# gargatik/Seamless-Through-Breaking-Rethinking-Image-Stitching-for-Optimal-Alignment

Hardware: AMD Instinct MI355X
Metric: stitched image-pairs/s at 512x512 (higher is better)
Workload: dtype f32 (decoder contractions, PatchEmbed's third conv and the C = 128 block tails: exact 3xbf16 split of both operands, 6 products on the bf16 matrix cores, fp32 accumulate -- error vs fp64 0.83x the fp32 MFMA chain's; everything else fp32); 1 GPU; UDIS-D-shaped 512x512 pairs, batch=1, FlowHomoAdpater.forward(type=test_eval); launch=hipGraph replay, pairs_in_flight=3

## Files before the change

include/stitch_gfx950.h:

```cpp
#ifndef STITCH_GFX950_H
#define STITCH_GFX950_H
#include <stdint.h>
#ifdef __cplusplus
extern "C" {
#endif

typedef struct st_gemm_desc {
    const float* a;
    const float* w;
    float* c;
    const float* bias;
    const float* aux0;
    const float* aux1;
    const float* aux2;
    const float* scale_ptr;
    int32_t M, N, K;
    int32_t H, W, Cin, ldx;
    int32_t kh, kw, sh, sw, ph, pw, Ho, Wo;
    int32_t ldw, ldc, ld_aux0, ld_aux1, ld_aux2;
    int32_t aux0_row_div, aux0_row_mod;
    int32_t act;
    int32_t epi;
    float alpha;
    int32_t batch;
// ... 130 lines not shown
int st_coords_grid_init(float* out, const float* init, int32_t B, int32_t H, int32_t W, void* stream);
int st_flow_forward_interpolate(const float* src, int32_t src_is_coords_rows, float* out, int32_t B, int32_t H, int32_t W,
                                void* stream);
int st_flow_from_coords(const float* coords1, float* flow4, int32_t ld4, float* dst2, int32_t ld2, int32_t B,
                        int32_t H, int32_t W, void* stream);
int st_flow_encode(const float* coords1, const float* w98, const float* bias, float* out, int32_t ldo, float* flow2,
                   int32_t ld2, int32_t B, int32_t H, int32_t W, int32_t Co, void* stream);
int st_flow_encode_split3(const float* coords1, const float* w98, const float* bias, float* out, int32_t ldo, float* flow2,
                          int32_t ld2, int32_t B, int32_t H, int32_t W, int32_t Co, void* out_planes, int64_t out_pstride,
                          int64_t out_prows, void* flow_planes, int64_t flow_pstride, int64_t flow_prows, int32_t flow_col,
                          void* stream);
int st_cost_lookup(const float* maps, const float* coords, float* out, int32_t ldo, int32_t Nq, int32_t H2,
                   int32_t W2, int32_t r, void* stream);
int st_decoder_token_chain(float* corr, int32_t ld_corr, const float* coords1, const float* kv,
                           const float* const* weights16, int32_t rows, int32_t ntok, void* stream);
int st_convex_upsample(const float* coords1, const float* mask, int32_t ldm, float* out, int32_t B, int32_t H,
                       int32_t W, void* stream);

int st_dlt4(const float* src4x2, const float* motion, float* H, int32_t B, float mscale_x, float mscale_y,
            float div, void* stream);
int st_mat3_sandwich(const float* L, const float* X, const float* R, float* out, int32_t B, int32_t invert,
                     void* stream);
int st_homo_warp(const float* U, const float* theta, float* out, int32_t* idx, int32_t B, int32_t C,
                 int32_t n_ones, int32_t H, int32_t W, int32_t oh, int32_t ow, void* stream);
int st_mesh_bounds(const float* H, float* out4, int32_t B, float width, float height, int32_t gw, int32_t gh,
                   void* stream);
int st_flow_warp(const float* x, const float* flow, const float* mul, float* out, int32_t B, int32_t C,
                 int32_t H, int32_t W, void* stream);
int st_homo_flow_warp(const float* image2, const float* H8, const float* flow, float* out6, float* overlap, float* Hi,
                      int32_t B, int32_t H, int32_t W, void* stream);
// ... 133 lines not shown
```

seamless-through-breaking-rethinking-image-stitching-for-optimal-alignment_amd/csrc/flowops.hip:

```cpp
#include "common.h"
#include <type_traits>
#include "../../include/stitch_gfx950.h"

__global__ void coords_grid_kernel(float* __restrict__ out, int B, int H, int W) {
    const size_t idx = (size_t)blockIdx.x * blockDim.x + threadIdx.x;
    if (idx >= (size_t)B * H * W) return;
    const int r = idx % ((size_t)H * W);
    out[idx * 2] = (float)(r % W);
    out[idx * 2 + 1] = (float)(r / W);
}

extern "C" int st_coords_grid(float* out, int32_t B, int32_t H, int32_t W, void* stream) {
    if (!out || B <= 0 || H <= 0 || W <= 0) return ST_EINVAL;
    const size_t total = (size_t)B * H * W;
    hipLaunchKernelGGL(coords_grid_kernel, dim3((total + 255) / 256), dim3(256), 0, (hipStream_t)stream, out, B, H, W);
    ST_CHECK_LAUNCH();
    return ST_OK;
}

__global__ void coords_grid_init_kernel(float* __restrict__ out, const float* __restrict__ init, int B, int H, int W) {
    const size_t idx = (size_t)blockIdx.x * blockDim.x + threadIdx.x;
    if (idx >= (size_t)B * H * W) return;
    const size_t N = (size_t)H * W, b = idx / N;
    const int r = idx % N;
// ... 21 lines not shown
        for (int c = 2; c < ld4; ++c) flow4[idx * ld4 + c] = 0.f;
    }
    if (dst2) { dst2[idx * ld2] = fx; dst2[idx * ld2 + 1] = fy; }
}

extern "C" int st_flow_from_coords(const float* coords1, float* flow4, int32_t ld4, float* dst2, int32_t ld2, int32_t B,
                                   int32_t H, int32_t W, void* stream) {
    if (!coords1 || B <= 0 || H <= 0 || W <= 0 || (flow4 && ld4 < 2) || (dst2 && ld2 < 2)) return ST_EINVAL;
    const size_t total = (size_t)B * H * W;
    hipLaunchKernelGGL(flow_from_coords_kernel, dim3((total + 255) / 256), dim3(256), 0, (hipStream_t)stream, coords1, flow4,
                       ld4, dst2, ld2, B, H, W);
    ST_CHECK_LAUNCH();
    return ST_OK;
}

__global__ __launch_bounds__(512) void flow_encode_kernel(const float* __restrict__ coords1, const float* __restrict__ w,
                                                          const float* __restrict__ bias, float* __restrict__ out, int ldo,
                                                          float* __restrict__ flow2, int ld2, int H, int W, int Co,
                                                          __bf16* __restrict__ out_planes, long long out_pstride, long long out_prows,
                                                          __bf16* __restrict__ flow_planes, long long flow_pstride, long long flow_prows, int flow_col) {
    __shared__ float2 patch[10 * 14];
    __shared__ __attribute__((aligned(16))) float wsm[98 * 128];
    const int tid = threadIdx.x, lane = tid & 63, wave = __builtin_amdgcn_readfirstlane(tid >> 6);
    const int tiles_x = (W + 7) >> 3;
    const int b = blockIdx.z, ty = (int)blockIdx.x / tiles_x, tx = (int)blockIdx.x - ty * tiles_x;
    const size_t img = (size_t)b * H * W;
    const int cbase = (int)blockIdx.y * 128;
    {
        float4 v[7];
#pragma unroll
        for (int u = 0; u < 7; ++u) {
            const int f = u * 512 + tid, t = f >> 5, c4 = (f & 31) * 4;
            v[u] = make_float4(0.f, 0.f, 0.f, 0.f);
            if (t < 98 && cbase + c4 < Co) v[u] = *reinterpret_cast<const float4*>(w + (size_t)t * Co + cbase + c4);
        }
#pragma unroll
        for (int u = 0; u < 7; ++u) {
            const int f = u * 512 + tid;
            if (f < 98 * 32) *reinterpret_cast<float4*>(wsm + f * 4) = v[u];
        }
    }
    if (tid < 140) {
        const int py = tid / 14, px = tid - py * 14;
        const int y = ty * 4 + py - 3, x = tx * 8 + px - 3;
        float2 f = make_float2(0.f, 0.f);
        if (y >= 0 && y < H && x >= 0 && x < W) {
            const float2 cc = *reinterpret_cast<const float2*>(coords1 + (img + (size_t)y * W + x) * 2);
            f = make_float2(cc.x - (float)x, cc.y - (float)y);
        }
        patch[tid] = f;
    }
    __syncthreads();
    const int row = wave >> 1;
    const int y = ty * 4 + row;
    if (y >= H) return;
    const int cl = (wave & 1) * 64 + lane, c = cbase + cl;
    const bool cok = c < Co;
    const float bv = cok ? bias[c] : 0.f;
    float acc[8];
#pragma unroll
    for (int p = 0; p < 8; ++p) acc[p] = bv;
#pragma unroll 1
    for (int ky = 0; ky < 7; ++ky) {
        float2 f[14];
        float wr[14];
#pragma unroll
        for (int i = 0; i < 14; ++i) {
            f[i] = patch[(row + ky) * 14 + i];
            wr[i] = wsm[(ky * 14 + i) * 128 + cl];
        }
#pragma unroll
        for (int kx = 0; kx < 7; ++kx)
#pragma unroll
            for (int p = 0; p < 8; ++p) {
                acc[p] = fmaf(f[p + kx].x, wr[kx * 2], acc[p]);
                acc[p] = fmaf(f[p + kx].y, wr[kx * 2 + 1], acc[p]);
            }
    }
#pragma unroll
    for (int p = 0; p < 8; ++p) {
        const int x = tx * 8 + p;
        if (x < W && cok) {
            const float o = fmaxf(acc[p], 0.f);
            out[(img + (size_t)y * W + x) * ldo + c] = o;
            if (out_planes) {
                __bf16 h, m, l;
                st_split3(o, h, m, l);
                const unsigned ph = st_bf16_bits(h), pm = st_bf16_bits(m), pl = st_bf16_bits(l);
                const unsigned nh = (unsigned)__builtin_amdgcn_update_dpp(0, (int)ph, 0xB1, 0xF, 0xF, false);
                const unsigned nm = (unsigned)__builtin_amdgcn_update_dpp(0, (int)pm, 0xB1, 0xF, 0xF, false);
                const unsigned nl = (unsigned)__builtin_amdgcn_update_dpp(0, (int)pl, 0xB1, 0xF, 0xF, false);
                if (!(c & 1)) {
                    unsigned* pp = reinterpret_cast<unsigned*>(out_planes + ((size_t)(c >> 5) * out_prows + img + (size_t)y * W + x) * 32 + (c & 31));
                    pp[0] = ph | (nh << 16); pp[out_pstride / 2] = pm | (nm << 16); pp[out_pstride] = pl | (nl << 16);
                }
            }
        }
    }
    if (flow2 && blockIdx.y == 0 && (wave & 1) == 0 && lane < 8 && tx * 8 + lane < W) {
        const float2 f = patch[(row + 3) * 14 + lane + 3];
        const size_t r = img + (size_t)y * W + tx * 8 + lane;
        flow2[r * ld2] = f.x; flow2[r * ld2 + 1] = f.y;
        if (flow_planes) {
            __bf16 hx, mx, lx, hy, my, ly;
            unsigned* pp = reinterpret_cast<unsigned*>(flow_planes + ((size_t)(flow_col >> 5) * flow_prows + r) * 32 + (flow_col & 31));
            st_split3(f.x, hx, mx, lx);
            st_split3(f.y, hy, my, ly);
            pp[0] = st_bf16_bits(hx) | ((unsigned)st_bf16_bits(hy) << 16);
            pp[flow_pstride / 2] = st_bf16_bits(mx) | ((unsigned)st_bf16_bits(my) << 16);
            pp[flow_pstride] = st_bf16_bits(lx) | ((unsigned)st_bf16_bits(ly) << 16);
        }
    }
}

extern "C" int st_flow_encode(const float* coords1, const float* w98, const float* bias, float* out, int32_t ldo, float* flow2,
                              int32_t ld2, int32_t B, int32_t H, int32_t W, int32_t Co, void* stream) {
    if (!coords1 || !w98 || !bias || !out || B <= 0 || H <= 0 || W <= 0 || Co <= 0 || (Co & 3) || ((uintptr_t)w98 & 15)) return ST_EINVAL;
    if (ldo < Co || (flow2 && ld2 < 2) || ((uintptr_t)coords1 & 7)) return ST_EINVAL;
    dim3 grid(((H + 3) / 4) * ((W + 7) / 8), (Co + 127) / 128, B);
    hipLaunchKernelGGL(flow_encode_kernel, grid, dim3(512), 0, (hipStream_t)stream, coords1, w98, bias, out, ldo, flow2, ld2, H, W, Co,
                       (__bf16*)nullptr, 0LL, 0LL, (__bf16*)nullptr, 0LL, 0LL, 0);
    ST_CHECK_LAUNCH();
    return ST_OK;
}

extern "C" int st_flow_encode_split3(const float* coords1, const float* w98, const float* bias, float* out, int32_t ldo, float* flow2,
                                     int32_t ld2, int32_t B, int32_t H, int32_t W, int32_t Co, void* out_planes, int64_t out_pstride,
                                     int64_t out_prows, void* flow_planes, int64_t flow_pstride, int64_t flow_prows, int32_t flow_col,
                                     void* stream) {
    if (!coords1 || !w98 || !bias || !out || B <= 0 || H <= 0 || W <= 0 || Co <= 0 || (Co & 31) || ((uintptr_t)w98 & 15)) return ST_EINVAL;
    if (ldo < Co || (flow2 && ld2 < 2) || ((uintptr_t)coords1 & 7)) return ST_EINVAL;
    if (!out_planes || out_pstride <= 0 || out_prows < (int64_t)B * H * W) return ST_EINVAL;
    if (flow_planes && (!flow2 || flow_pstride <= 0 || flow_prows < (int64_t)B * H * W || flow_col < 0 || (flow_col & 1))) return ST_EINVAL;
    dim3 grid(((H + 3) / 4) * ((W + 7) / 8), (Co + 127) / 128, B);
    hipLaunchKernelGGL(flow_encode_kernel, grid, dim3(512), 0, (hipStream_t)stream, coords1, w98, bias, out, ldo, flow2, ld2, H, W, Co,
                       (__bf16*)out_planes, (long long)out_pstride, (long long)out_prows, (__bf16*)flow_planes, (long long)flow_pstride,
                       (long long)flow_prows, (int)flow_col);
    ST_CHECK_LAUNCH();
    return ST_OK;
}

__global__ __launch_bounds__(256) void cost_lookup_kernel(const float* __restrict__ maps, const float* __restrict__ coords,
                                                          float* __restrict__ out, int ldo, int Nq, int H2, int W2, int r) {
#pragma clang fp contract(off)
    const int side = 2 * r + 1, nch = side * side;
    const size_t idx = (size_t)blockIdx.x * 256 + threadIdx.x;
    if (idx >= (size_t)Nq * nch) return;
    const int ch = idx % nch;
    const size_t n = idx / nch;
    const int i = ch / side, j = ch % side;
    const float x = coords[n * 2] + (float)(i - r);
    const float y = coords[n * 2 + 1] + (float)(j - r);
    const float gx = 2.0f * x / (float)(W2 - 1) - 1.0f, gy = 2.0f * y / (float)(H2 - 1) - 1.0f;
    const float ix = ((gx + 1.0f) / 2.0f) * (float)(W2 - 1), iy = ((gy + 1.0f) / 2.0f) * (float)(H2 - 1);
    const float x0f = floorf(ix), y0f = floorf(iy);
    const int x0 = (int)x0f, y0 = (int)y0f, x1 = x0 + 1, y1 = y0 + 1;
    const float x1f = x0f + 1.0f, y1f = y0f + 1.0f;
    const float nw = (x1f - ix) * (y1f - iy), ne = (ix - x0f) * (y1f - iy);
    const float sw = (x1f - ix) * (iy - y0f), se = (ix - x0f) * (iy - y0f);
    const float* m = maps + n * (size_t)(H2 * W2);
    const bool xin0 = x0 >= 0 && x0 < W2, xin1 = x1 >= 0 && x1 < W2;
    const bool yin0 = y0 >= 0 && y0 < H2, yin1 = y1 >= 0 && y1 < H2;
    float v = (xin0 && yin0 ? m[y0 * W2 + x0] : 0.f) * nw;
    v = __fmaf_rn(xin1 && yin0 ? m[y0 * W2 + x1] : 0.f, ne, v);
    v = __fmaf_rn(xin0 && yin1 ? m[y1 * W2 + x0] : 0.f, sw, v);
    v = __fmaf_rn(xin1 && yin1 ? m[y1 * W2 + x1] : 0.f, se, v);
    out[n * ldo + ch] = v;
}

extern "C" int st_cost_lookup(const float* maps, const float* coords, float* out, int32_t ldo, int32_t Nq, int32_t H2,
                              int32_t W2, int32_t r, void* stream) {
    if (!maps || !coords || !out || Nq <= 0 || r < 0 || r > 64 || ldo < (2 * r + 1) * (2 * r + 1)) return ST_EINVAL;
    if (H2 < 2 || W2 < 2 || (int64_t)H2 * W2 > 0x7fffffff) return ST_EINVAL;
    const size_t total = (size_t)Nq * (2 * r + 1) * (2 * r + 1);
    hipLaunchKernelGGL(cost_lookup_kernel, dim3((total + 255) / 256), dim3(256), 0, (hipStream_t)stream, maps, coords, out,
                       ldo, Nq, H2, W2, r);
    ST_CHECK_LAUNCH();
    return ST_OK;
}

__global__ __launch_bounds__(256) void convex_upsample_kernel(const float* __restrict__ coords1, const float* __restrict__ mask,
                                                              int ldm, float* __restrict__ out, int B, int H, int W) {
// ... 98 lines not shown
    for (int r = 0; r < 4; ++r) {
        const float mo = red_other[(4 * g + r) * 2], m2o = red_other[(4 * g + r) * 2 + 1];
        const float mean = 0.5f * (mh[r] + mo), d = mh[r] - mo;
        const float var = ((m2h[r] + m2o) + d * d * 16.0f) * (1.0f / 64.0f);
        const float rstd = 1.0f / sqrtf(var + 1e-5f);
#pragma unroll
        for (int t = 0; t < 2; ++t) v[t][r] = (v[t][r] - mean) * rstd * w[col0 + 16 * t + c] + b[col0 + 16 * t + c];
    }
}

template <int I, int N, class F>
__device__ __forceinline__ void tc_static_for(F&& f) {
    if constexpr (I < N) { f(std::integral_constant<int, I>{}); tc_static_for<I + 1, N>(f); }
}

template <int RG>
__global__ __launch_bounds__(128 * RG) void decoder_token_chain_kernel(float* __restrict__ corr, int ldc, const float* __restrict__ coords1,
                                                                       const float* __restrict__ kv, TokenChainArgs A, int rows, int ntok) {
    extern __shared__ __attribute__((aligned(16))) float sm[];
    float* W0 = sm;
    float* W2 = W0 + 64 * TC_LDW0;
    float* Wq = W2 + 64 * TC_LDW;
    float* Wp = Wq + 64 * TC_LDW;
    float* Wf0 = Wp + 64 * TC_LDW;
    float* Wf3 = Wf0 + 64 * TC_LDW;
    float* Vec = Wf3 + 64 * TC_LDW;
    float* Slab = Vec + 10 * 64;
    float* Red = Slab + RG * 16 * (TC_LDW0 + TC_LDW);
    const int tid = threadIdx.x, lane = tid & 63, wave = tid >> 6;
    constexpr int NT = 128 * RG;
    const int rg = wave >> 1, hf = wave & 1, col0 = 32 * hf;
    float* S0 = Slab + rg * 16 * (TC_LDW0 + TC_LDW);
    float* S1 = S0 + 16 * TC_LDW0;
    float* red_mine = Red + (rg * 2 + hf) * 32;
    const float* red_other = Red + (rg * 2 + (hf ^ 1)) * 32;
    const int row0 = (blockIdx.x * RG + rg) * 16;
    const int c = lane & 15, g = lane >> 4;
    const int jmax = ntok - 1;

    constexpr int P0 = 1536 / NT, P1 = 1024 / NT;
    float4 xv[3], w0v[P0];
    f32x4 wv[5 * P1], vecv;
    float cx[4], cy[4];
    {
        const int e = min(tid, 159), q = e >> 4;
        const float* vp = q == 0 ? A.b0 : q == 1 ? A.b2 : q == 2 ? A.n1w : q == 3 ? A.n1b : q == 4 ? A.bq : q == 5 ? A.bp : q == 6 ? A.n2w
                          : q == 7 ? A.n2b : q == 8 ? A.bf0 : A.bf3;
        vecv = *reinterpret_cast<const f32x4*>(vp + 4 * (e & 15));
    }
    tc_static_for<0, 3>([&](auto ic) {
        constexpr int i = decltype(ic)::value;
        const int e = (hf * 64 + lane) + 128 * i, r = e / 24, k4 = e % 24;
        xv[i] = *reinterpret_cast<const float4*>(corr + (size_t)min(row0 + r, rows - 1) * ldc + 4 * min(k4, 20));
    });
    tc_static_for<0, P0>([&](auto ic) {
        constexpr int i = decltype(ic)::value;
        const int e = tid + NT * i, n = e / 24, k4 = e % 24;
        w0v[i] = *reinterpret_cast<const float4*>(A.w0 + n * 84 + 4 * min(k4, 20));
    });
    tc_static_for<0, P1>([&](auto ic) {
        constexpr int i = decltype(ic)::value;
        const int off = 4 * (tid + NT * i);
        wv[5 * i + 0] = *reinterpret_cast<const f32x4*>(A.w2 + off);
        wv[5 * i + 1] = *reinterpret_cast<const f32x4*>(A.wq + off);
        wv[5 * i + 2] = *reinterpret_cast<const f32x4*>(A.wp + off);
        wv[5 * i + 3] = *reinterpret_cast<const f32x4*>(A.wf0 + off);
        wv[5 * i + 4] = *reinterpret_cast<const f32x4*>(A.wf3 + off);
    });
#pragma unroll
    for (int r = 0; r < 4; ++r) {
        const float2 p2 = *reinterpret_cast<const float2*>(coords1 + (size_t)min(row0 + 4 * g + r, rows - 1) * 2);
        cx[r] = p2.x; cy[r] = p2.y;
    }
    tc_static_for<0, 3>([&](auto ic) {
        constexpr int i = decltype(ic)::value;
        const int e = (hf * 64 + lane) + 128 * i, r = e / 24, k4 = e % 24;
        *reinterpret_cast<float4*>(S0 + r * TC_LDW0 + 4 * k4) = k4 < 21 ? xv[i] : make_float4(0.f, 0.f, 0.f, 0.f);
    });
    tc_static_for<0, P0>([&](auto ic) {
        constexpr int i = decltype(ic)::value;
        const int e = tid + NT * i, n = e / 24, k4 = e % 24;
        *reinterpret_cast<float4*>(W0 + n * TC_LDW0 + 4 * k4) = k4 < 21 ? w0v[i] : make_float4(0.f, 0.f, 0.f, 0.f);
    });
    tc_static_for<0, P1>([&](auto ic) {
        constexpr int i = decltype(ic)::value;
        const int e = tid + NT * i, n = e >> 4, k4 = e & 15, off = n * TC_LDW + 4 * k4;
        *reinterpret_cast<f32x4*>(W2 + off) = wv[5 * i + 0];
        *reinterpret_cast<f32x4*>(Wq + off) = wv[5 * i + 1];
        *reinterpret_cast<f32x4*>(Wp + off) = wv[5 * i + 2];
        *reinterpret_cast<f32x4*>(Wf0 + off) = wv[5 * i + 3];
        *reinterpret_cast<f32x4*>(Wf3 + off) = wv[5 * i + 4];
    });
    if (tid < 160) *reinterpret_cast<f32x4*>(Vec + 4 * tid) = vecv;
    asm volatile("" ::: "memory");
    const int head = 4 * hf + g;
    float4 kk[8][2], vv[8][2];
    {
        const float* kvr = kv + (size_t)min(row0 + c, rows - 1) * ntok * 128 + 8 * head;
#pragma unroll
        for (int j = 0; j < 8; ++j)
#pragma unroll
            for (int e = 0; e < 2; ++e) kk[j][e] = *reinterpret_cast<const float4*>(kvr + min(j, jmax) * 128 + 4 * e);
#pragma unroll
        for (int j = 0; j < 8; ++j)
#pragma unroll
            for (int e = 0; e < 2; ++e) vv[j][e] = *reinterpret_cast<const float4*>(kvr + min(j, jmax) * 128 + 64 + 4 * e);
    }
    asm volatile("" ::: "memory");
// ... 82 lines not shown
    for (int t = 0; t < 2; ++t)
#pragma unroll
        for (int r = 0; r < 4; ++r) acc[t][r] = st_act(acc[t][r] + bf0[col0 + 16 * t + c], ST_ACT_GELU);
    tc_store2(S1, acc, col0, lane);
    __syncthreads();
    tc_gemm2<64, TC_LDW, TC_LDW>(S1, Wf3 + col0 * TC_LDW, acc, lane);
#pragma unroll
    for (int t = 0; t < 2; ++t)
#pragma unroll
        for (int r = 0; r < 4; ++r) {
            const int row = row0 + 4 * g + r;
            if (row < rows) corr[(size_t)row * ldc + 84 + col0 + 16 * t + c] = x[t][r] + (acc[t][r] + bf3[col0 + 16 * t + c]);
        }
}

extern "C" int st_decoder_token_chain(float* corr, int32_t ld_corr, const float* coords1, const float* kv, const float* const* weights16,
                                      int32_t rows, int32_t ntok, void* stream) {
    if (!corr || !coords1 || !kv || !weights16 || rows <= 0 || ntok <= 0 || ntok > 8 || ld_corr < 148 || (ld_corr & 3)) return ST_EINVAL;
    TokenChainArgs A;
    const float** dst = reinterpret_cast<const float**>(&A);
    for (int i = 0; i < 16; ++i) { if (!weights16[i]) return ST_EINVAL; dst[i] = weights16[i]; }
    constexpr int RG = 4;
    const size_t lds = (size_t)(64 * TC_LDW0 + 5 * 64 * TC_LDW + 640 + RG * 16 * (TC_LDW0 + TC_LDW) + RG * 64) * sizeof(float);
    (void)hipFuncSetAttribute((const void*)decoder_token_chain_kernel<RG>, hipFuncAttributeMaxDynamicSharedMemorySize, (int)lds);
    hipLaunchKernelGGL(decoder_token_chain_kernel<RG>, dim3((rows + 16 * RG - 1) / (16 * RG)), dim3(128 * RG), lds, (hipStream_t)stream, corr, ld_corr,
                       coords1, kv, A, rows, ntok);
    ST_CHECK_LAUNCH();
    return ST_OK;
}
```

seamless-through-breaking-rethinking-image-stitching-for-optimal-alignment_amd/flowformer.py:

```python
from __future__ import annotations

import os

import torch
import torch.nn as nn

from . import ops
from .checkpoint import HP, ParamTree, flat_params, flow_spec
from .homography import pack_conv


SPLIT3 = os.environ.get("ST_SPLIT3", "1") != "0"


def _new(rows, cols, dev, zero=False):
    return (torch.zeros if zero else torch.empty)((rows, cols), device=dev, dtype=torch.float32)


def _planes_copy(p):
    return ops.Planes(p.rows, p.C, None, t=p.t.clone(), c0=p.c0, ncols=p.ncols)


def _keep(trace, **named):
    if trace is None:
# ... 451 lines not shown
        for sfx in ("1", "2"):
            tabs[sfx] = _new(inp.shape[0], 384, inp.device)
            ops.conv_gemm(inp, D["inp" + sfx][0], tabs[sfx], geom=gru_geom[sfx], bias=D["inp" + sfx][1])
        return tabs

    def _update_state(self, R, B, N, dev):
        S = dict(hxA=_new(R, 384, dev), hxB=_new(R, 384, dev), corr=_new(R, 160, dev, zero=True),
                 cor1=_new(R, 256, dev), corflo=_new(R, 256, dev), flo1=_new(R, 128, dev),
                 vT=torch.empty((B, 128, N), device=dev), zbuf=_new(R, 128, dev), fh=_new(R, 256, dev))
        S["s3"] = SPLIT3 and N % 32 == 0 and "s3" in self._pk["dec"]
        if S["s3"]:
            S.update(hxA_p=ops.Planes(R, 384, dev), hxB_p=ops.Planes(R, 384, dev), cor1_p=ops.Planes(R, 256, dev), flo1_p=ops.Planes(R, 128, dev),
                     corflo_p=ops.Planes(R, 256, dev))
        return S

    def _update_block(self, S, coords1, attn, gru_tab, B, H1, W1, trace=None):
        D = self._pk["dec"]
        N = H1 * W1
        s3 = S["s3"]
        hxA = S["hxA"]
        net, motion, flow, agg = hxA[:, :128], hxA[:, 128:254], hxA[:, 254:256], hxA[:, 256:]
        g3 = (B, H1, W1, 3, 3, 1, 1, 1, 1)
        _keep(trace, coords_in=coords1, net_in=net)
        ops.conv_gemm(S["corr"], D["convc1"][0], S["cor1"], bias=D["convc1"][1], act="relu", **_emit(S, "cor1", 0, 256))
        enc = (coords1, D["convf1"][0], D["convf1"][1], S["flo1"], flow, B, H1, W1)
        if s3:
            ops.flow_encode_split3(*enc, S["flo1_p"], (S["hxA_p"], 254))
        else:
            ops.flow_encode(*enc)
        ops.conv_gemm_pair((_act(S, "cor1", 0, 256), _wt(D, S, "convc2"), S["corflo"][:, :192],
                            dict(geom=g3, bias=D["convc2"][1], act="relu", **_emit(S, "corflo", 0, 192, no_f32=True))),
                           (_act(S, "flo1", 0, 128), _wt(D, S, "convf2"), S["corflo"][:, 192:],
                            dict(geom=g3, bias=D["convf2"][1], act="relu", **_emit(S, "corflo", 192, 256, no_f32=True))))
        corflo = _act(S, "corflo", 0, 256)
        _keep(trace, cor1=S["cor1"], flo1=S["flo1"], flow=flow, **{"corflo_p" if s3 else "corflo": corflo})
        ops.conv_gemm(corflo, _wt(D, S, "conv"), motion, geom=g3, bias=D["conv"][1], act="relu", **_emit(S, "hxA", 128, 256))
        _keep(trace, motion=motion)
        ops.gma_aggregate(attn, hxA[:, 128:256], D["to_v"], D["gamma"], S["vT"], agg, B, N, **_emit(S, "hxA", 256, 384))
        _keep(trace, aggregate=agg)
        gru = (S["zbuf"], gru_tab["1"], gru_tab["2"], *((D["s3"] if s3 else D)[k] for k in ("zr1", "q1", "zr2", "q2")), B, H1, W1)
        if s3:
            ops.sepconv_gru_split3(hxA, S["hxA_p"], S["hxB_p"], *gru)
        else:
            ops.sepconv_gru(hxA, S["hxB"], *gru)
# ... 33 lines not shown
    def _decoder(self, mem, ctx, cost_maps, B, H1, W1, iters, trace=None, flow_init=None):
        D = self._pk["dec"]
        dev = ctx.device
        N = H1 * W1
        R = B * N
        nl = self._pk["latents"].shape[0]
        pro = None if trace is None else trace[-1].setdefault("prologue", {})
        pre = self._decoder_prologue(ctx, B, H1, W1, trace=pro)
        S, gru_tab, attn = pre["S"], pre["gru_tab"], pre["attn"]
        kv = _new(R * nl, 128, dev)
        ops.conv_gemm(mem, D["ca"]["kv"][0], kv, bias=D["ca"]["kv"][1])
        _keep(pro, kv=kv)
        coords1 = _new(R, 2, dev)
        ops.coords_grid(coords1, B, H1, W1, init=flow_init)
        for it in range(iters):
            ops.cost_lookup9x9(cost_maps, coords1, S["corr"], R, H1, W1)
            ops.decoder_token_chain(S["corr"], coords1, kv, D["chain16"], R, nl)
            rec = _record(trace)
            self._update_block(S, coords1, attn, gru_tab, B, H1, W1, trace=rec)
            _keep(rec, coords1=coords1, net=S["hxA"][:, :128], corr=S["corr"])
        last = None if trace is None else trace[-1]
        mask = self._mask_head(S, B, H1, W1, trace=last)
        flow_up = torch.empty((B, 2, 8 * H1, 8 * W1), device=dev)
        ops.convex_upsample(coords1, mask, flow_up, B, H1, W1)
        _keep(last, mask=mask, flow_up=flow_up)
        return flow_up, coords1

    def _forward(self, image1, image2, iters, trace, flow_init, pair):
        if not image1.is_cuda:
            raise RuntimeError("FlowFormer runs on the MI355X HIP kernels only: move the module and inputs to cuda")
        pk = self._pk or self.pack()
        iters = HP["decoder_depth"] if iters is None else iters
        B, _, H, W = image1.shape
        if H % 32 or W % 32:
            raise RuntimeError(f"input size {H}x{W} must be a multiple of 32 (reference runs both nets at 512x512)")
# ... 44 lines not shown
```

seamless-through-breaking-rethinking-image-stitching-for-optimal-alignment_amd/ops.py:

```python
from __future__ import annotations

import ctypes as C

import torch

from ._lib import ChainDesc, GemmDesc, MlpDesc, check, lib
from ._lib import StitchError as StitchErrorBase

ACT = dict(none=0, relu=1, gelu=2, sigmoid=3, tanh=4, lrelu=5)
EPI = dict(store=0, add=1, mul=2, gru=3, axpy=4, zr=5)

assert lib.st_abi_gemm_desc_size() == C.sizeof(GemmDesc), "st_gemm_desc ABI mismatch between header and binding"
assert lib.st_abi_chain_desc_size() == C.sizeof(ChainDesc), "st_chain_desc ABI mismatch between header and binding"
assert lib.st_abi_mlp_desc_size() == C.sizeof(MlpDesc), "st_mlp_desc ABI mismatch between header and binding"


def _stream():
    return C.c_void_p(torch.cuda.current_stream().cuda_stream)


def _p(t):
    if t is None:
        return None
    assert t.is_cuda, "device tensor expected (no CPU fallback)"
# ... 404 lines not shown
                                    C.c_void_p(fp.t.data_ptr()), fp.pstride, fp.rows, int(fcol), _stream()), "st_flow_encode_split3")
    return out


def cost_lookup(maps, coords, out, Nq, H2, W2, r=4):
    check(lib.st_cost_lookup(_p(maps), _p(coords), _p(out), _ld(out), Nq, H2, W2, r, _stream()), "st_cost_lookup")
    return out


def decoder_token_chain(corr, coords1, kv, weights16, rows, ntok):
    arr = (C.c_void_p * 16)(*[w.data_ptr() for w in weights16])
    check(lib.st_decoder_token_chain(_p(corr), _ld(corr), _pc(coords1), _p(kv), arr, rows, ntok, _stream()), "st_decoder_token_chain")
    return corr


def _ws(dev):
    ws = _workspace(dev)
    return ws.data_ptr(), ws.numel()


def patch_conv12(maps, c0_w, c0_b, c2_w, c2_b, out, M, H=64, W=64):
    check(lib.st_patch_conv12(_pc(maps), _pc(c0_w), _pc(c0_b), _pc(c2_w), _pc(c2_b), _p(out), M, H, W, _stream()), "st_patch_conv12")
    return out


def cost_lookup9x9(maps, coords, out, Nq, H2, W2):
    check(lib.st_cost_lookup9x9(_p(maps), _pc(coords), _p(out), _ld(out), Nq, H2, W2, _stream()), "st_cost_lookup9x9")
    return out


# ... 625 lines not shown
```

Baseline: 93.94 pairs/s.

## Fuse cost lookup, token chain and flow encode into one decoder-front kernel

```diff
diff --git a/include/stitch_gfx950.h b/include/stitch_gfx950.h
--- a/include/stitch_gfx950.h
+++ b/include/stitch_gfx950.h
@@ -168,6 +168,10 @@
                    int32_t W2, int32_t r, void* stream);
 int st_decoder_token_chain(float* corr, int32_t ld_corr, const float* coords1, const float* kv,
                            const float* const* weights16, int32_t rows, int32_t ntok, void* stream);
+int st_decoder_front(const float* cost_maps, const float* coords1, float* corr, int32_t ld_corr, const float* kv,
+                     const float* const* weights16, int32_t ntok, const float* w98, const float* bias, float* flo1, int32_t ld_flo1,
+                     float* flow2, int32_t ld2, int32_t B, int32_t H, int32_t W, void* flo1_planes, int64_t flo1_pstride,
+                     int64_t flo1_prows, void* flow_planes, int64_t flow_pstride, int64_t flow_prows, int32_t flow_col, void* stream);
 int st_convex_upsample(const float* coords1, const float* mask, int32_t ldm, float* out, int32_t B, int32_t H,
                        int32_t W, void* stream);
 
diff --git a/seamless-through-breaking-rethinking-image-stitching-for-optimal-alignment_amd/csrc/flowops.hip b/seamless-through-breaking-rethinking-image-stitching-for-optimal-alignment_amd/csrc/flowops.hip
--- a/seamless-through-breaking-rethinking-image-stitching-for-optimal-alignment_amd/csrc/flowops.hip
+++ b/seamless-through-breaking-rethinking-image-stitching-for-optimal-alignment_amd/csrc/flowops.hip
@@ -59,33 +59,33 @@
     return ST_OK;
 }
 
-__global__ __launch_bounds__(512) void flow_encode_kernel(const float* __restrict__ coords1, const float* __restrict__ w,
-                                                          const float* __restrict__ bias, float* __restrict__ out, int ldo,
-                                                          float* __restrict__ flow2, int ld2, int H, int W, int Co,
-                                                          __bf16* __restrict__ out_planes, long long out_pstride, long long out_prows,
-                                                          __bf16* __restrict__ flow_planes, long long flow_pstride, long long flow_prows, int flow_col) {
-    __shared__ float2 patch[10 * 14];
-    __shared__ __attribute__((aligned(16))) float wsm[98 * 128];
-    const int tid = threadIdx.x, lane = tid & 63, wave = __builtin_amdgcn_readfirstlane(tid >> 6);
-    const int tiles_x = (W + 7) >> 3;
-    const int b = blockIdx.z, ty = (int)blockIdx.x / tiles_x, tx = (int)blockIdx.x - ty * tiles_x;
-    const size_t img = (size_t)b * H * W;
-    const int cbase = (int)blockIdx.y * 128;
-    {
-        float4 v[7];
-#pragma unroll
-        for (int u = 0; u < 7; ++u) {
-            const int f = u * 512 + tid, t = f >> 5, c4 = (f & 31) * 4;
-            v[u] = make_float4(0.f, 0.f, 0.f, 0.f);
-            if (t < 98 && cbase + c4 < Co) v[u] = *reinterpret_cast<const float4*>(w + (size_t)t * Co + cbase + c4);
-        }
-#pragma unroll
-        for (int u = 0; u < 7; ++u) {
-            const int f = u * 512 + tid;
-            if (f < 98 * 32) *reinterpret_cast<float4*>(wsm + f * 4) = v[u];
-        }
-    }
+struct FlowEncArgs {
+    const float *w, *bias;
+    float* out; int ldo;
+    float* flow2; int ld2;
+    int H, W, Co;
+    __bf16* out_planes; long long out_pstride, out_prows;
+    __bf16* flow_planes; long long flow_pstride, flow_prows; int flow_col;
+};
+
+__device__ __forceinline__ void fe_stage_weights(float* __restrict__ wsm, const float* __restrict__ w, int cbase, int Co, int tid) {
+    float4 v[7];
+#pragma unroll
+    for (int u = 0; u < 7; ++u) {
+        const int f = u * 512 + tid, t = f >> 5, c4 = (f & 31) * 4;
+        v[u] = make_float4(0.f, 0.f, 0.f, 0.f);
+        if (t < 98 && cbase + c4 < Co) v[u] = *reinterpret_cast<const float4*>(w + (size_t)t * Co + cbase + c4);
+    }
+#pragma unroll
+    for (int u = 0; u < 7; ++u) {
+        const int f = u * 512 + tid;
+        if (f < 98 * 32) *reinterpret_cast<float4*>(wsm + f * 4) = v[u];
+    }
+}
+
+__device__ __forceinline__ void fe_stage_patch(float2* __restrict__ patch, const float* __restrict__ coords1, int b, int ty, int tx, int H, int W, int tid) {
     if (tid < 140) {
+        const size_t img = (size_t)b * H * W;
         const int py = tid / 14, px = tid - py * 14;
         const int y = ty * 4 + py - 3, x = tx * 8 + px - 3;
         float2 f = make_float2(0.f, 0.f);
@@ -95,13 +95,19 @@
         }
         patch[tid] = f;
     }
-    __syncthreads();
+}
+
+__device__ __forceinline__ void fe_tile(const float2* __restrict__ patch, const float* __restrict__ wsm, const FlowEncArgs& F, int b, int ty, int tx,
+                                        int cbase, int tid) {
+    const int lane = tid & 63, wave = __builtin_amdgcn_readfirstlane(tid >> 6);
+    const int H = F.H, W = F.W, Co = F.Co, ldo = F.ldo;
+    const size_t img = (size_t)b * H * W;
     const int row = wave >> 1;
     const int y = ty * 4 + row;
     if (y >= H) return;
     const int cl = (wave & 1) * 64 + lane, c = cbase + cl;
     const bool cok = c < Co;
-    const float bv = cok ? bias[c] : 0.f;
+    const float bv = cok ? F.bias[c] : 0.f;
     float acc[8];
 #pragma unroll
     for (int p = 0; p < 8; ++p) acc[p] = bv;
@@ -127,8 +133,8 @@
         const int x = tx * 8 + p;
         if (x < W && cok) {
             const float o = fmaxf(acc[p], 0.f);
-            out[(img + (size_t)y * W + x) * ldo + c] = o;
-            if (out_planes) {
+            F.out[(img + (size_t)y * W + x) * ldo + c] = o;
+            if (F.out_planes) {
                 __bf16 h, m, l;
                 st_split3(o, h, m, l);
                 const unsigned ph = st_bf16_bits(h), pm = st_bf16_bits(m), pl = st_bf16_bits(l);
@@ -136,26 +142,39 @@
                 const unsigned nm = (unsigned)__builtin_amdgcn_update_dpp(0, (int)pm, 0xB1, 0xF, 0xF, false);
                 const unsigned nl = (unsigned)__builtin_amdgcn_update_dpp(0, (int)pl, 0xB1, 0xF, 0xF, false);
                 if (!(c & 1)) {
-                    unsigned* pp = reinterpret_cast<unsigned*>(out_planes + ((size_t)(c >> 5) * out_prows + img + (size_t)y * W + x) * 32 + (c & 31));
-                    pp[0] = ph | (nh << 16); pp[out_pstride / 2] = pm | (nm << 16); pp[out_pstride] = pl | (nl << 16);
+                    unsigned* pp = reinterpret_cast<unsigned*>(F.out_planes + ((size_t)(c >> 5) * F.out_prows + img + (size_t)y * W + x) * 32 + (c & 31));
+                    pp[0] = ph | (nh << 16); pp[F.out_pstride / 2] = pm | (nm << 16); pp[F.out_pstride] = pl | (nl << 16);
                 }
             }
         }
     }
-    if (flow2 && blockIdx.y == 0 && (wave & 1) == 0 && lane < 8 && tx * 8 + lane < W) {
+    if (F.flow2 && cbase == 0 && (wave & 1) == 0 && lane < 8 && tx * 8 + lane < W) {
         const float2 f = patch[(row + 3) * 14 + lane + 3];
         const size_t r = img + (size_t)y * W + tx * 8 + lane;
-        flow2[r * ld2] = f.x; flow2[r * ld2 + 1] = f.y;
-        if (flow_planes) {
+        F.flow2[r * F.ld2] = f.x; F.flow2[r * F.ld2 + 1] = f.y;
+        if (F.flow_planes) {
             __bf16 hx, mx, lx, hy, my, ly;
-            unsigned* pp = reinterpret_cast<unsigned*>(flow_planes + ((size_t)(flow_col >> 5) * flow_prows + r) * 32 + (flow_col & 31));
+            unsigned* pp = reinterpret_cast<unsigned*>(F.flow_planes + ((size_t)(F.flow_col >> 5) * F.flow_prows + r) * 32 + (F.flow_col & 31));
             st_split3(f.x, hx, mx, lx);
             st_split3(f.y, hy, my, ly);
             pp[0] = st_bf16_bits(hx) | ((unsigned)st_bf16_bits(hy) << 16);
-            pp[flow_pstride / 2] = st_bf16_bits(mx) | ((unsigned)st_bf16_bits(my) << 16);
-            pp[flow_pstride] = st_bf16_bits(lx) | ((unsigned)st_bf16_bits(ly) << 16);
-        }
-    }
+            pp[F.flow_pstride / 2] = st_bf16_bits(mx) | ((unsigned)st_bf16_bits(my) << 16);
+            pp[F.flow_pstride] = st_bf16_bits(lx) | ((unsigned)st_bf16_bits(ly) << 16);
+        }
+    }
+}
+
+__global__ __launch_bounds__(512) void flow_encode_kernel(const float* __restrict__ coords1, FlowEncArgs F) {
+    __shared__ float2 patch[10 * 14];
+    __shared__ __attribute__((aligned(16))) float wsm[98 * 128];
+    const int tid = threadIdx.x;
+    const int tiles_x = (F.W + 7) >> 3;
+    const int b = blockIdx.z, ty = (int)blockIdx.x / tiles_x, tx = (int)blockIdx.x - ty * tiles_x;
+    const int cbase = (int)blockIdx.y * 128;
+    fe_stage_weights(wsm, F.w, cbase, F.Co, tid);
+    fe_stage_patch(patch, coords1, b, ty, tx, F.H, F.W, tid);
+    __syncthreads();
+    fe_tile(patch, wsm, F, b, ty, tx, cbase, tid);
 }
 
 extern "C" int st_flow_encode(const float* coords1, const float* w98, const float* bias, float* out, int32_t ldo, float* flow2,
@@ -163,8 +182,8 @@
     if (!coords1 || !w98 || !bias || !out || B <= 0 || H <= 0 || W <= 0 || Co <= 0 || (Co & 3) || ((uintptr_t)w98 & 15)) return ST_EINVAL;
     if (ldo < Co || (flow2 && ld2 < 2) || ((uintptr_t)coords1 & 7)) return ST_EINVAL;
     dim3 grid(((H + 3) / 4) * ((W + 7) / 8), (Co + 127) / 128, B);
-    hipLaunchKernelGGL(flow_encode_kernel, grid, dim3(512), 0, (hipStream_t)stream, coords1, w98, bias, out, ldo, flow2, ld2, H, W, Co,
-                       (__bf16*)nullptr, 0LL, 0LL, (__bf16*)nullptr, 0LL, 0LL, 0);
+    const FlowEncArgs F{w98, bias, out, ldo, flow2, ld2, H, W, Co, nullptr, 0, 0, nullptr, 0, 0, 0};
+    hipLaunchKernelGGL(flow_encode_kernel, grid, dim3(512), 0, (hipStream_t)stream, coords1, F);
     ST_CHECK_LAUNCH();
     return ST_OK;
 }
@@ -178,39 +197,57 @@
     if (!out_planes || out_pstride <= 0 || out_prows < (int64_t)B * H * W) return ST_EINVAL;
     if (flow_planes && (!flow2 || flow_pstride <= 0 || flow_prows < (int64_t)B * H * W || flow_col < 0 || (flow_col & 1))) return ST_EINVAL;
     dim3 grid(((H + 3) / 4) * ((W + 7) / 8), (Co + 127) / 128, B);
-    hipLaunchKernelGGL(flow_encode_kernel, grid, dim3(512), 0, (hipStream_t)stream, coords1, w98, bias, out, ldo, flow2, ld2, H, W, Co,
-                       (__bf16*)out_planes, (long long)out_pstride, (long long)out_prows, (__bf16*)flow_planes, (long long)flow_pstride,
-                       (long long)flow_prows, (int)flow_col);
-    ST_CHECK_LAUNCH();
-    return ST_OK;
+    const FlowEncArgs F{w98, bias, out, ldo, flow2, ld2, H, W, Co, (__bf16*)out_planes, (long long)out_pstride, (long long)out_prows,
+                        (__bf16*)flow_planes, (long long)flow_pstride, (long long)flow_prows, (int)flow_col};
+    hipLaunchKernelGGL(flow_encode_kernel, grid, dim3(512), 0, (hipStream_t)stream, coords1, F);
+    ST_CHECK_LAUNCH();
+    return ST_OK;
+}
+
+struct LookupTaps {
+    int x0, y0;
+    float nw, ne, sw, se;
+};
+
+__device__ __forceinline__ LookupTaps lookup_taps(float cx, float cy, int di, int dj, int H2, int W2) {
+#pragma clang fp contract(off)
+    const float x = cx + (float)di;
+    const float y = cy + (float)dj;
+    const float gx = 2.0f * x / (float)(W2 - 1) - 1.0f, gy = 2.0f * y / (float)(H2 - 1) - 1.0f;
+    const float ix = ((gx + 1.0f) / 2.0f) * (float)(W2 - 1), iy = ((gy + 1.0f) / 2.0f) * (float)(H2 - 1);
+    const float x0f = floorf(ix), y0f = floorf(iy);
+    const float x1f = x0f + 1.0f, y1f = y0f + 1.0f;
+    LookupTaps t;
+    t.x0 = (int)x0f; t.y0 = (int)y0f;
+    t.nw = (x1f - ix) * (y1f - iy); t.ne = (ix - x0f) * (y1f - iy);
+    t.sw = (x1f - ix) * (iy - y0f); t.se = (ix - x0f) * (iy - y0f);
+    return t;
+}
+
+__device__ __forceinline__ float lookup_blend(float vnw, float vne, float vsw, float vse, const LookupTaps& t) {
+#pragma clang fp contract(off)
+    float v = vnw * t.nw;
+    v = __fmaf_rn(vne, t.ne, v);
+    v = __fmaf_rn(vsw, t.sw, v);
+    v = __fmaf_rn(vse, t.se, v);
+    return v;
 }
 
 __global__ __launch_bounds__(256) void cost_lookup_kernel(const float* __restrict__ maps, const float* __restrict__ coords,
                                                           float* __restrict__ out, int ldo, int Nq, int H2, int W2, int r) {
-#pragma clang fp contract(off)
     const int side = 2 * r + 1, nch = side * side;
     const size_t idx = (size_t)blockIdx.x * 256 + threadIdx.x;
     if (idx >= (size_t)Nq * nch) return;
     const int ch = idx % nch;
     const size_t n = idx / nch;
     const int i = ch / side, j = ch % side;
-    const float x = coords[n * 2] + (float)(i - r);
-    const float y = coords[n * 2 + 1] + (float)(j - r);
-    const float gx = 2.0f * x / (float)(W2 - 1) - 1.0f, gy = 2.0f * y / (float)(H2 - 1) - 1.0f;
-    const float ix = ((gx + 1.0f) / 2.0f) * (float)(W2 - 1), iy = ((gy + 1.0f) / 2.0f) * (float)(H2 - 1);
-    const float x0f = floorf(ix), y0f = floorf(iy);
-    const int x0 = (int)x0f, y0 = (int)y0f, x1 = x0 + 1, y1 = y0 + 1;
-    const float x1f = x0f + 1.0f, y1f = y0f + 1.0f;
-    const float nw = (x1f - ix) * (y1f - iy), ne = (ix - x0f) * (y1f - iy);
-    const float sw = (x1f - ix) * (iy - y0f), se = (ix - x0f) * (iy - y0f);
+    const LookupTaps t = lookup_taps(coords[n * 2], coords[n * 2 + 1], i - r, j - r, H2, W2);
+    const int x0 = t.x0, y0 = t.y0, x1 = x0 + 1, y1 = y0 + 1;
     const float* m = maps + n * (size_t)(H2 * W2);
     const bool xin0 = x0 >= 0 && x0 < W2, xin1 = x1 >= 0 && x1 < W2;
     const bool yin0 = y0 >= 0 && y0 < H2, yin1 = y1 >= 0 && y1 < H2;
-    float v = (xin0 && yin0 ? m[y0 * W2 + x0] : 0.f) * nw;
-    v = __fmaf_rn(xin1 && yin0 ? m[y0 * W2 + x1] : 0.f, ne, v);
-    v = __fmaf_rn(xin0 && yin1 ? m[y1 * W2 + x0] : 0.f, sw, v);
-    v = __fmaf_rn(xin1 && yin1 ? m[y1 * W2 + x1] : 0.f, se, v);
-    out[n * ldo + ch] = v;
+    out[n * ldo + ch] = lookup_blend(xin0 && yin0 ? m[y0 * W2 + x0] : 0.f, xin1 && yin0 ? m[y0 * W2 + x1] : 0.f,
+                                     xin0 && yin1 ? m[y1 * W2 + x0] : 0.f, xin1 && yin1 ? m[y1 * W2 + x1] : 0.f, t);
 }
 
 extern "C" int st_cost_lookup(const float* maps, const float* coords, float* out, int32_t ldo, int32_t Nq, int32_t H2,
@@ -339,10 +376,10 @@
     if constexpr (I < N) { f(std::integral_constant<int, I>{}); tc_static_for<I + 1, N>(f); }
 }
 
-template <int RG>
-__global__ __launch_bounds__(128 * RG) void decoder_token_chain_kernel(float* __restrict__ corr, int ldc, const float* __restrict__ coords1,
-                                                                       const float* __restrict__ kv, TokenChainArgs A, int rows, int ntok) {
-    extern __shared__ __attribute__((aligned(16))) float sm[];
+template <int RG, bool LOOKUP>
+__device__ __forceinline__ void tc_body(float* __restrict__ sm, int wg, float* __restrict__ corr, int ldc, const float* __restrict__ coords1,
+                                        const float* __restrict__ kv, const TokenChainArgs& A, int rows, int ntok, const float* __restrict__ maps,
+                                        int mapH, int mapW) {
     float* W0 = sm;
     float* W2 = W0 + 64 * TC_LDW0;
     float* Wq = W2 + 64 * TC_LDW;
@@ -359,7 +396,7 @@
     float* S1 = S0 + 16 * TC_LDW0;
     float* red_mine = Red + (rg * 2 + hf) * 32;
     const float* red_other = Red + (rg * 2 + (hf ^ 1)) * 32;
-    const int row0 = (blockIdx.x * RG + rg) * 16;
+    const int row0 = (wg * RG + rg) * 16;
     const int c = lane & 15, g = lane >> 4;
     const int jmax = ntok - 1;
 
@@ -367,13 +404,24 @@
     float4 xv[3], w0v[P0];
     f32x4 wv[5 * P1], vecv;
     float cx[4], cy[4];
+    constexpr int LK = 11;
+    static_assert(!LOOKUP || NT == 8 * 16 * RG, "the lookup gives 8 threads to each of the workgroup's rows");
+    const int lrow = tid >> 3, lc0 = tid & 7;
+    const int lgrow = min(wg * RG * 16 + lrow, rows - 1);
+    float2 lxy = make_float2(0.f, 0.f);
+    if constexpr (LOOKUP) lxy = *reinterpret_cast<const float2*>(coords1 + (size_t)lgrow * 2);
+#pragma unroll
+    for (int r = 0; r < 4; ++r) {
+        const float2 p2 = *reinterpret_cast<const float2*>(coords1 + (size_t)min(row0 + 4 * g + r, rows - 1) * 2);
+        cx[r] = p2.x; cy[r] = p2.y;
+    }
     {
         const int e = min(tid, 159), q = e >> 4;
         const float* vp = q == 0 ? A.b0 : q == 1 ? A.b2 : q == 2 ? A.n1w : q == 3 ? A.n1b : q == 4 ? A.bq : q == 5 ? A.bp : q == 6 ? A.n2w
                           : q == 7 ? A.n2b : q == 8 ? A.bf0 : A.bf3;
         vecv = *reinterpret_cast<const f32x4*>(vp + 4 * (e & 15));
     }
-    tc_static_for<0, 3>([&](auto ic) {
+    if constexpr (!LOOKUP) tc_static_for<0, 3>([&](auto ic) {
         constexpr int i = decltype(ic)::value;
         const int e = (hf * 64 + lane) + 128 * i, r = e / 24, k4 = e % 24;
         xv[i] = *reinterpret_cast<const float4*>(corr + (size_t)min(row0 + r, rows - 1) * ldc + 4 * min(k4, 20));
@@ -392,12 +440,20 @@
         wv[5 * i + 3] = *reinterpret_cast<const f32x4*>(A.wf0 + off);
         wv[5 * i + 4] = *reinterpret_cast<const f32x4*>(A.wf3 + off);
     });
-#pragma unroll
-    for (int r = 0; r < 4; ++r) {
-        const float2 p2 = *reinterpret_cast<const float2*>(coords1 + (size_t)min(row0 + 4 * g + r, rows - 1) * 2);
-        cx[r] = p2.x; cy[r] = p2.y;
-    }
-    tc_static_for<0, 3>([&](auto ic) {
+    float tap[LK][4];
+    if constexpr (LOOKUP) {
+        const float* m = maps + (size_t)lgrow * (size_t)(mapH * mapW);
+        tc_static_for<0, LK>([&](auto kc) {
+            constexpr int k = decltype(kc)::value;
+            const int ch = min(lc0 + 8 * k, 80);
+            const LookupTaps t = lookup_taps(lxy.x, lxy.y, ch / 9 - 4, ch % 9 - 4, mapH, mapW);
+            const int xa = min(max(t.x0, 0), mapW - 1), xb = min(max(t.x0, -1), mapW - 2) + 1;
+            const int ya = min(max(t.y0, 0), mapH - 1), yb = min(max(t.y0, -1), mapH - 2) + 1;
+            tap[k][0] = m[ya * mapW + xa]; tap[k][1] = m[ya * mapW + xb];
+            tap[k][2] = m[yb * mapW + xa]; tap[k][3] = m[yb * mapW + xb];
+        });
+    }
+    if constexpr (!LOOKUP) tc_static_for<0, 3>([&](auto ic) {
         constexpr int i = decltype(ic)::value;
         const int e = (hf * 64 + lane) + 128 * i, r = e / 24, k4 = e % 24;
         *reinterpret_cast<float4*>(S0 + r * TC_LDW0 + 4 * k4) = k4 < 21 ? xv[i] : make_float4(0.f, 0.f, 0.f, 0.f);
@@ -417,6 +473,23 @@
         *reinterpret_cast<f32x4*>(Wf3 + off) = wv[5 * i + 4];
     });
     if (tid < 160) *reinterpret_cast<f32x4*>(Vec + 4 * tid) = vecv;
+    if constexpr (LOOKUP) {
+        float* Srow = Slab + (lrow >> 4) * 16 * (TC_LDW0 + TC_LDW) + (lrow & 15) * TC_LDW0;
+        const bool live = wg * RG * 16 + lrow < rows;
+        tc_static_for<0, LK>([&](auto kc) {
+            constexpr int k = decltype(kc)::value;
+            const int chr = lc0 + 8 * k, ch = min(chr, 80);
+            const LookupTaps t = lookup_taps(lxy.x, lxy.y, ch / 9 - 4, ch % 9 - 4, mapH, mapW);
+            const int x0 = t.x0, y0 = t.y0, x1 = x0 + 1, y1 = y0 + 1;
+            const bool xin0 = x0 >= 0 && x0 < mapW, xin1 = x1 >= 0 && x1 < mapW;
+            const bool yin0 = y0 >= 0 && y0 < mapH, yin1 = y1 >= 0 && y1 < mapH;
+            const float v = lookup_blend(xin0 && yin0 ? tap[k][0] : 0.f, xin1 && yin0 ? tap[k][1] : 0.f, xin0 && yin1 ? tap[k][2] : 0.f,
+                                         xin1 && yin1 ? tap[k][3] : 0.f, t);
+            Srow[chr] = chr < 81 ? v : 0.f;
+            if (live && chr < 81) corr[(size_t)lgrow * ldc + chr] = v;
+        });
+        Srow[88 + lc0] = 0.f;
+    }
     asm volatile("" ::: "memory");
     const int head = 4 * hf + g;
     float4 kk[8][2], vv[8][2];
@@ -529,6 +602,18 @@
         }
 }
 
+template <int RG>
+__global__ __launch_bounds__(128 * RG) void decoder_token_chain_kernel(float* __restrict__ corr, int ldc, const float* __restrict__ coords1,
+                                                                       const float* __restrict__ kv, TokenChainArgs A, int rows, int ntok) {
+    extern __shared__ __attribute__((aligned(16))) float sm[];
+    tc_body<RG, false>(sm, (int)blockIdx.x, corr, ldc, coords1, kv, A, rows, ntok, nullptr, 0, 0);
+}
+
+template <int RG>
+static constexpr size_t tc_lds_bytes() {
+    return (size_t)(64 * TC_LDW0 + 5 * 64 * TC_LDW + 640 + RG * 16 * (TC_LDW0 + TC_LDW) + RG * 64) * sizeof(float);
+}
+
 extern "C" int st_decoder_token_chain(float* corr, int32_t ld_corr, const float* coords1, const float* kv, const float* const* weights16,
                                       int32_t rows, int32_t ntok, void* stream) {
     if (!corr || !coords1 || !kv || !weights16 || rows <= 0 || ntok <= 0 || ntok > 8 || ld_corr < 148 || (ld_corr & 3)) return ST_EINVAL;
@@ -536,10 +621,62 @@
     const float** dst = reinterpret_cast<const float**>(&A);
     for (int i = 0; i < 16; ++i) { if (!weights16[i]) return ST_EINVAL; dst[i] = weights16[i]; }
     constexpr int RG = 4;
-    const size_t lds = (size_t)(64 * TC_LDW0 + 5 * 64 * TC_LDW + 640 + RG * 16 * (TC_LDW0 + TC_LDW) + RG * 64) * sizeof(float);
+    const size_t lds = tc_lds_bytes<RG>();
     (void)hipFuncSetAttribute((const void*)decoder_token_chain_kernel<RG>, hipFuncAttributeMaxDynamicSharedMemorySize, (int)lds);
     hipLaunchKernelGGL(decoder_token_chain_kernel<RG>, dim3((rows + 16 * RG - 1) / (16 * RG)), dim3(128 * RG), lds, (hipStream_t)stream, corr, ld_corr,
                        coords1, kv, A, rows, ntok);
     ST_CHECK_LAUNCH();
     return ST_OK;
 }
+
+#define DF_TILES_PER_WG 4
+
+__global__ __launch_bounds__(512) void decoder_front_kernel(float* __restrict__ corr, int ldc, const float* __restrict__ coords1,
+                                                            const float* __restrict__ kv, TokenChainArgs A, int rows, int ntok,
+                                                            const float* __restrict__ maps, FlowEncArgs F, int B, int row_wgs) {
+    extern __shared__ __attribute__((aligned(16))) float sm[];
+    if ((int)blockIdx.x < row_wgs) {
+        tc_body<4, true>(sm, (int)blockIdx.x, corr, ldc, coords1, kv, A, rows, ntok, maps, F.H, F.W);
+        return;
+    }
+    float* wsm = sm;
+    float2* patch = reinterpret_cast<float2*>(sm + 98 * 128);
+    const int tid = threadIdx.x;
+    const int tiles_x = (F.W + 7) >> 3, per_img = tiles_x * ((F.H + 3) >> 2), total = per_img * B;
+    const int step = (int)gridDim.x - row_wgs;
+    fe_stage_weights(wsm, F.w, 0, F.Co, tid);
+    int buf = 0;
+    for (int t = (int)blockIdx.x - row_wgs; t < total; t += step, buf ^= 1) {
+        const int b = t / per_img, rem = t - b * per_img, ty = rem / tiles_x, tx = rem - ty * tiles_x;
+        fe_stage_patch(patch + buf * 140, coords1, b, ty, tx, F.H, F.W, tid);
+        __syncthreads();
+        fe_tile(patch + buf * 140, wsm, F, b, ty, tx, 0, tid);
+    }
+}
+
+extern "C" int st_decoder_front(const float* cost_maps, const float* coords1, float* corr, int32_t ld_corr, const float* kv,
+                                const float* const* weights16, int32_t ntok, const float* w98, const float* bias, float* flo1, int32_t ld_flo1,
+                                float* flow2, int32_t ld2, int32_t B, int32_t H, int32_t W, void* flo1_planes, int64_t flo1_pstride,
+                                int64_t flo1_prows, void* flow_planes, int64_t flow_pstride, int64_t flow_prows, int32_t flow_col, void* stream) {
+    if (!cost_maps || !coords1 || !corr || !kv || !weights16 || !w98 || !bias || !flo1 || !flow2) return ST_EINVAL;
+    if (B <= 0 || H < 2 || W < 2 || (int64_t)B * H * W > 0x7fffffff || (int64_t)H * W > 0x7fffffff) return ST_EINVAL;
+    if (ntok <= 0 || ntok > 8 || ld_corr < 160 || (ld_corr & 3) || ld_flo1 < 128 || ld2 < 2) return ST_EINVAL;
+    if (((uintptr_t)coords1 & 7) || ((uintptr_t)w98 & 15) || ((uintptr_t)corr & 15) || ((uintptr_t)kv & 15)) return ST_EINVAL;
+    const int rows = B * H * W;
+    if (flo1_planes && (flo1_pstride <= 0 || flo1_prows < rows)) return ST_EINVAL;
+    if (flow_planes && (flow_pstride <= 0 || flow_prows < rows || flow_col < 0 || (flow_col & 1))) return ST_EINVAL;
+    TokenChainArgs A;
+    const float** dst = reinterpret_cast<const float**>(&A);
+    for (int i = 0; i < 16; ++i) { if (!weights16[i] || ((uintptr_t)weights16[i] & 15)) return ST_EINVAL; dst[i] = weights16[i]; }
+    const FlowEncArgs F{w98, bias, flo1, ld_flo1, flow2, ld2, H, W, 128, (__bf16*)flo1_planes, (long long)flo1_pstride, (long long)flo1_prows,
+                        (__bf16*)flow_planes, (long long)flow_pstride, (long long)flow_prows, (int)flow_col};
+    const int row_wgs = (rows + 63) / 64;
+    const int tiles = B * ((H + 3) / 4) * ((W + 7) / 8), flow_wgs = (tiles + DF_TILES_PER_WG - 1) / DF_TILES_PER_WG;
+    const size_t lds = tc_lds_bytes<4>();
+    static_assert(tc_lds_bytes<4>() >= (98 * 128 + 2 * 140 * 2) * sizeof(float), "the flow workgroups' weights and patches fit the chain's LDS");
+    (void)hipFuncSetAttribute((const void*)decoder_front_kernel, hipFuncAttributeMaxDynamicSharedMemorySize, (int)lds);
+    hipLaunchKernelGGL(decoder_front_kernel, dim3(row_wgs + flow_wgs), dim3(512), lds, (hipStream_t)stream, corr, ld_corr, coords1, kv, A, rows,
+                       ntok, cost_maps, F, B, row_wgs);
+    ST_CHECK_LAUNCH();
+    return ST_OK;
+}
diff --git a/seamless-through-breaking-rethinking-image-stitching-for-optimal-alignment_amd/flowformer.py b/seamless-through-breaking-rethinking-image-stitching-for-optimal-alignment_amd/flowformer.py
--- a/seamless-through-breaking-rethinking-image-stitching-for-optimal-alignment_amd/flowformer.py
+++ b/seamless-through-breaking-rethinking-image-stitching-for-optimal-alignment_amd/flowformer.py
@@ -489,6 +489,17 @@
                      corflo_p=ops.Planes(R, 256, dev))
         return S
 
+    def _iteration(self, S, coords1, cost_maps, kv, attn, gru_tab, B, H1, W1, trace=None):
+        D = self._pk["dec"]
+        s3 = S["s3"]
+        ops.decoder_front(cost_maps, coords1, S["corr"], kv, D["chain16"], self._pk["latents"].shape[0], D["convf1"][0], D["convf1"][1],
+                          S["flo1"], S["hxA"][:, 254:256], B, H1, W1, flo1_planes=S["flo1_p"] if s3 else None,
+                          flow_planes=(S["hxA_p"], 254) if s3 else None)
+        rec = _record(trace)
+        self._update_block(S, coords1, attn, gru_tab, B, H1, W1, trace=rec)
+        _keep(rec, coords1=coords1, net=S["hxA"][:, :128], corr=S["corr"])
+        return rec
+
     def _update_block(self, S, coords1, attn, gru_tab, B, H1, W1, trace=None):
         D = self._pk["dec"]
         N = H1 * W1
@@ -498,11 +509,6 @@
         g3 = (B, H1, W1, 3, 3, 1, 1, 1, 1)
         _keep(trace, coords_in=coords1, net_in=net)
         ops.conv_gemm(S["corr"], D["convc1"][0], S["cor1"], bias=D["convc1"][1], act="relu", **_emit(S, "cor1", 0, 256))
-        enc = (coords1, D["convf1"][0], D["convf1"][1], S["flo1"], flow, B, H1, W1)
-        if s3:
-            ops.flow_encode_split3(*enc, S["flo1_p"], (S["hxA_p"], 254))
-        else:
-            ops.flow_encode(*enc)
         ops.conv_gemm_pair((_act(S, "cor1", 0, 256), _wt(D, S, "convc2"), S["corflo"][:, :192],
                             dict(geom=g3, bias=D["convc2"][1], act="relu", **_emit(S, "corflo", 0, 192, no_f32=True))),
                            (_act(S, "flo1", 0, 128), _wt(D, S, "convf2"), S["corflo"][:, 192:],
@@ -566,11 +572,7 @@
         coords1 = _new(R, 2, dev)
         ops.coords_grid(coords1, B, H1, W1, init=flow_init)
         for it in range(iters):
-            ops.cost_lookup9x9(cost_maps, coords1, S["corr"], R, H1, W1)
-            ops.decoder_token_chain(S["corr"], coords1, kv, D["chain16"], R, nl)
-            rec = _record(trace)
-            self._update_block(S, coords1, attn, gru_tab, B, H1, W1, trace=rec)
-            _keep(rec, coords1=coords1, net=S["hxA"][:, :128], corr=S["corr"])
+            self._iteration(S, coords1, cost_maps, kv, attn, gru_tab, B, H1, W1, trace=trace)
         last = None if trace is None else trace[-1]
         mask = self._mask_head(S, B, H1, W1, trace=last)
         flow_up = torch.empty((B, 2, 8 * H1, 8 * W1), device=dev)
diff --git a/seamless-through-breaking-rethinking-image-stitching-for-optimal-alignment_amd/ops.py b/seamless-through-breaking-rethinking-image-stitching-for-optimal-alignment_amd/ops.py
--- a/seamless-through-breaking-rethinking-image-stitching-for-optimal-alignment_amd/ops.py
+++ b/seamless-through-breaking-rethinking-image-stitching-for-optimal-alignment_amd/ops.py
@@ -442,6 +442,18 @@
     return corr
 
 
+def decoder_front(cost_maps, coords1, corr, kv, weights16, ntok, w98, bias, flo1, flow2, B, H, W, flo1_planes=None, flow_planes=None):
+    arr = (C.c_void_p * 16)(*[w.data_ptr() for w in weights16])
+    fp, fcol = flow_planes if flow_planes is not None else (None, 0)
+    check(lib.st_decoder_front(_pc(cost_maps), _pc(coords1), _p(corr), _ld(corr), _pc(kv), arr, ntok, _pc(w98), _pc(bias), _p(flo1), _ld(flo1),
+                               _p(flow2), _ld(flow2), B, H, W,
+                               C.c_void_p(flo1_planes.ptr()) if flo1_planes is not None else None,
+                               flo1_planes.pstride if flo1_planes is not None else 0, flo1_planes.rows if flo1_planes is not None else 0,
+                               C.c_void_p(fp.t.data_ptr()) if fp is not None else None, fp.pstride if fp is not None else 0,
+                               fp.rows if fp is not None else 0, int(fcol), _stream()), "st_decoder_front")
+    return corr
+
+
 def _ws(dev):
     ws = _workspace(dev)
     return ws.data_ptr(), ws.numel()
```

Result: no change. 94.11 pairs/s, median of 3 (+0.2%).
